# GothiProCoder/OCR-System

Hardware: AMD Instinct MI355X
Metric: pages/sec end-to-end det+rec, A4@200DPI (higher is better)
Workload: dtype bf16; 1 GPU; end-to-end det+rec, batch=64 A4@200DPI pages per GPU (BASELINE configs[3]); pages_per_gpu=64, global_batch=64, lines_last_step=3279, pages_gathered_last_step=64, parallelism=pages sharded dp1, 1 all-gather/step, ranks=1, input=pages pre-decoded (uint8 RGB) and resident in HBM when the timed region starts, det_sub_batch=64

## Files before the change

### ocr-system_amd/csrc/capi.hip

```cpp
#include <cstdlib>
#include <cstring>
#include <new>

#include "../../include/lumina_ocr.h"
#include "dbpost.h"
#include "deskew.h"
#include "engine.h"
#include "marks.h"
#include "barcodes.h"
#include "qrcodes.h"
#include "datamatrix.h"
#include "aztec.h"
#include "ops.h"
#include "orient.h"
#include "compose.h"
#include "resize.h"
#include "runs.h"
#include "jpeg.h"
#include "jpegdec.h"
#include "lzw.h"
#include "jp2dec.h"
#include "pngdec.h"
#include "vp8dec.h"
#include "webpdec.h"
// ... 94 lines not shown
    if (!eng) return 1;
    eng->device = device;
    int ndev = 0;
    if (hipGetDeviceCount(&ndev) != hipSuccess || device < 0 || device >= ndev) {
        eng->err = "no HIP device " + std::to_string(device) + " (device count " + std::to_string(ndev) + ")";
        *out = eng;
        return 2;
    }
    if (hipSetDevice(device) != hipSuccess) { eng->err = "hipSetDevice failed"; *out = eng; return 2; }
    if (const char* e = getenv("LUMINA_RING_ORIENT")) eng->ring_orient = atoi(e) < 0 ? -1 : (atoi(e) != 0);
    if (getenv("LUMINA_CONV_NO_RING")) eng->conv_ring = false;
    if (getenv("LUMINA_BLOCKED")) eng->blocked_layout = atoi(getenv("LUMINA_BLOCKED")) != 0;
    *out = eng;
    return 0;
}

void lumina_ocr_destroy(lumina_ocr_t* h) {
    if (!h) return;
    (void)hipSetDevice(h->device);
    delete h;
}

const char* lumina_ocr_last_error(const lumina_ocr_t* h) { return h ? h->err.c_str() : "null handle"; }

int lumina_ocr_set_option(lumina_ocr_t* h, const char* key, int value) {
    if (!h || !key) return 1;
    if (!strcmp(key, "det_sub_batch")) h->det_sub_batch = value > 0 ? value : 1;
    else if (!strcmp(key, "rec_sub_batch")) h->rec_sub_batch = value > 0 ? value : 1;
    else if (!strcmp(key, "cls_sub_batch")) h->cls_sub_batch = value > 0 ? value : 1;
    else if (!strcmp(key, "keep_taps")) h->keep_taps = value < 0 || value > 2 ? 0 : value;
    else if (!strcmp(key, "time_convs")) h->time_convs = value != 0;
    else if (!strcmp(key, "fuse_head")) h->fuse_head = value != 0;
    else if (!strcmp(key, "fuse_mb")) h->fuse_mb = value != 0;
    else if (!strcmp(key, "fuse_pool")) h->fuse_pool = value != 0;
    else if (!strcmp(key, "fuse_stem")) h->fuse_stem = value != 0;
    else if (!strcmp(key, "fpn_multi")) h->fpn_multi = value != 0;
    else if (!strcmp(key, "fpn_compose")) h->fpn_compose = value != 0;
    else if (!strcmp(key, "fuse_short")) h->fuse_short = value != 0;
    else if (!strcmp(key, "conv_ring")) h->conv_ring = value != 0;
    else if (!strcmp(key, "blocked_layout")) h->blocked_layout = value != 0;
    else if (!strcmp(key, "conv_big_min")) h->conv_big_min = value >= 0 ? value : 1024;
    else if (!strcmp(key, "ring_orient")) h->ring_orient = value < 0 ? -1 : (value != 0);
    else if (!strcmp(key, "post_group")) h->post_group = value > 0 ? value : 1;
    else if (!strcmp(key, "tail_group")) h->tail_group = value > 0 ? value : 0;
    else if (!strcmp(key, "svtr_f16")) h->svtr_f16 = value < 0 ? -1 : (value != 0);
    else if (!strcmp(key, "png_sub_batch_mb")) h->pd_sub_batch_mb = value > 0 ? value : 1;
    else if (!strcmp(key, "webp_sub_batch_mb")) h->wp_sub_batch_mb = value > 0 ? value : 1;
    else if (!strcmp(key, "jp2_sub_batch_mb")) h->jp_sub_batch_mb = value > 0 ? value : 1;
    else if (!strcmp(key, "conv2d_variant")) h->conv2d_variant = value < 0 || value > 2 ? 0 : value;
    else return locr_fail(h, "set_option: unknown key", key);
    return 0;
}

int lumina_ocr_load_det_weights(lumina_ocr_t* h, const void* blob, size_t nbytes) {
    if (!h || !blob) return 1;
    BIND(h);
    API_TRY return eng_load_det(h, blob, nbytes); API_CATCH(h)
}
int lumina_ocr_load_rec_weights(lumina_ocr_t* h, const void* blob, size_t nbytes) {
    if (!h || !blob) return 1;
    BIND(h);
    API_TRY return eng_load_rec(h, blob, nbytes); API_CATCH(h)
}
int lumina_ocr_num_classes(const lumina_ocr_t* h) { return h ? h->num_classes : 0; }

int lumina_ocr_normalize(lumina_ocr_t* h, const uint8_t* img_dev, int n, int height, int width, int hp, int wp, const float scale[3],
// ... 967 lines not shown
```

### ocr-system_amd/csrc/engine.h

```cpp
#pragma once
#include <map>
#include <memory>
#include <string>
#include <type_traits>
#include <vector>

#include "common.h"
#include "conv_mfma.h"
#include "mbconv.h"
#include "svtr.h"

struct Tensor4 {
    bf16_t* p = nullptr;
    int n = 0, h = 0, w = 0, c = 0;
    bool blk = false;
    int n_src = 0; const bf16_t* xs[4] = {nullptr, nullptr, nullptr, nullptr}; int xs_shift[4] = {0, 0, 0, 0};
    int xs_c[4] = {0, 0, 0, 0}, xs_cs[4] = {0, 0, 0, 0};
    int src_c(int k) const { return xs_c[k] ? xs_c[k] : c / n_src; }
    int src_cs(int k) const { return xs_cs[k] ? xs_cs[k] : src_c(k); }
    size_t elems() const { return (size_t)n * h * w * c; }
};

struct ConvLayer {
    std::string name;
// ... 49 lines not shown
inline hipError_t mem_alloc(PinnedMem* m, size_t bytes) { void* p = nullptr; hipError_t e = hipHostMalloc(&p, bytes, hipHostMallocDefault); m->reset(p); return e; }

template <class Mem> struct Growable {
    Mem mem;
    size_t cap = 0;
    uint8_t* get() const { return static_cast<uint8_t*>(mem.get()); }
    hipError_t reserve(size_t bytes, hipEvent_t in_use = nullptr) {
        if (bytes <= cap) return hipSuccess;
        hipError_t e = in_use ? hipEventSynchronize(in_use) : hipDeviceSynchronize();
        if (e != hipSuccess) return e;
        mem.reset(); cap = 0;
        if ((e = mem_alloc(&mem, bytes)) != hipSuccess) return e;
        cap = bytes;
        return hipSuccess;
    }
};

struct LaunchRecord { Event e0, e1; double flop, bytes; std::string layer, kernel; };

struct HostBlobTensor { int dtype; std::vector<int> dims; const uint8_t* data; size_t nbytes; };

struct lumina_ocr {
    int device = 0;
    std::string err;
    bool det_loaded = false;
    std::map<std::string, ConvLayer> det;
    bf16_t* stem_wpk = nullptr; float* stem_bias = nullptr;
    bool rec_loaded = false;
    int num_classes = 0, ctc_ntiles = 0;
    bf16_t* rstem_wpk = nullptr; float* rstem_bias = nullptr;
    std::vector<RecBlock> rblocks;
    ConvLayer rconv2, xproj[2];
    bf16_t* whh[2] = {nullptr, nullptr};
    bf16_t* ctc_wpk = nullptr; float* ctc_bias = nullptr;
    SvtrModel svtr;
    bool cls_loaded = false;
    bf16_t* cstem_wpk = nullptr; float* cstem_bias = nullptr;
    std::vector<RecBlock> cblocks;
    ConvLayer cconv2;
    float *cls_fc_w = nullptr, *cls_fc_b = nullptr;
    Growable<DeviceMem> ws;
    Arena arena;
    std::vector<DeviceMem> owned;
    bf16_t* zeros = nullptr;
    int det_sub_batch = 16, rec_sub_batch = 4096, cls_sub_batch = 4096, post_group = 64;
    int tail_group = 16;
    std::map<std::string, Tensor4> taps;
    int keep_taps = 0;
    bool fuse_head = true;
    bool fuse_pool = true;
    int conv_big_min = 1024;
    bool blocked_layout = true;
    bool conv_ring = true;
    int svtr_f16 = -1;
    int conv2d_variant = 0;
    int ring_orient = -1;
    bool fuse_short = true;
    bool fpn_compose = true;
    bool fpn_multi = true;
    bool fuse_stem = true;
    bool fuse_mb = true;
    bool time_convs = false;
    std::vector<LaunchRecord> launches;
    struct Coeffs { int ksize = 0; int* bounds = nullptr; int* kk = nullptr; std::shared_ptr<std::vector<int>> bounds_host; };
    std::map<std::pair<int, int>, Coeffs> coeff_cache;
    Growable<DeviceMem> aux;
    Growable<DeviceMem> sums;
    int jd_last_passes = 0;
    struct Staging { Growable<PinnedMem> buf; Event uploaded; };
    Staging jd_stage[2];
    int jd_stage_next = 0;
    Staging pd_stage;
    int pd_sub_batch_mb = 768;
    Staging jp_stage;
    Staging wp_stage;
    int wp_sub_batch_mb = 2048;
    int jp_sub_batch_mb = 4096;
    float* dk_trig = nullptr; short* dk_wtab = nullptr;
    Staging pc_stage;
    Growable<DeviceMem> pc_table;
};

int locr_fail(lumina_ocr* eng, const char* what, const char* detail);
bool parse_blob(lumina_ocr* eng, const void* blob, size_t n, std::map<std::string, HostBlobTensor>* out);

int eng_load_det(lumina_ocr* eng, const void* blob, size_t n);
int eng_load_rec(lumina_ocr* eng, const void* blob, size_t n);
int eng_det_forward(lumina_ocr* eng, const uint8_t* pages, int B, int H, int W, int Hp, int Wp, bf16_t* prob, hipStream_t st);
int eng_rec_forward(lumina_ocr* eng, const uint8_t* crops, const int* widths, int N, int* idx, float* prob, hipStream_t st);
int eng_load_svtr(lumina_ocr* eng, const void* blob, size_t n);
int eng_load_cls(lumina_ocr* eng, const void* blob, size_t n);
int eng_cls_forward(lumina_ocr* eng, const uint8_t* crops, const int* widths, int N, float thresh, int* label, float* score, int* flip, hipStream_t st);
int eng_svtr_forward(lumina_ocr* eng, const uint8_t* crops, const int* widths, int N, int* idx, float* prob, hipStream_t st);
int eng_ws_reserve(lumina_ocr* eng, size_t bytes);
// ... 19 lines not shown
```

### ocr-system_amd/csrc/engine.hip

```cpp
#include "engine.h"

#include <cstdlib>
#include <cstring>

#include "ops.h"
#include "stem_conv.h"

int locr_fail(lumina_ocr* eng, const char* what, const char* detail) {
    if (eng) eng->err = std::string(what) + ": " + (detail ? detail : "");
    return 1;
}

#define RUN(expr) do { if ((expr) != 0) return 1; } while (0)

#include <mutex>
#include <set>
hipError_t locr_dyn_lds(const void* kernel, int bytes) {
    static std::mutex mu;
    static std::set<std::pair<int, const void*>> done;
    int dev = 0;
    hipError_t e = hipGetDevice(&dev);
    if (e != hipSuccess) return e;
    std::lock_guard<std::mutex> lk(mu);
    if (done.count({dev, kernel})) return hipSuccess;
    e = hipFuncSetAttribute(kernel, hipFuncAttributeMaxDynamicSharedMemorySize, bytes);
    if (e == hipSuccess) done.insert({dev, kernel});
    return e;
}

bool parse_blob(lumina_ocr* eng, const void* blob, size_t n, std::map<std::string, HostBlobTensor>* out) {
    const uint8_t* b = static_cast<const uint8_t*>(blob);
    if (n < 12 || memcmp(b, "LOCW", 4) != 0) { locr_fail(eng, "parse_blob", "bad magic"); return false; }
    uint32_t ver, cnt;
    memcpy(&ver, b + 4, 4); memcpy(&cnt, b + 8, 4);
    if (ver != 1) { locr_fail(eng, "parse_blob", "unsupported version"); return false; }
    size_t off = 12;
    for (uint32_t i = 0; i < cnt; ++i) {
        if (off + 2 > n) { locr_fail(eng, "parse_blob", "truncated"); return false; }
// ... 591 lines not shown
        if (!make_dw(eng, m, p + ".dw", B.k, B.exp, cp16(B.exp), &B.dw)) return locr_fail(eng, "dw", p.c_str());
        {
            const HostBlobTensor *w, *b;
            if (!get_wb(eng, m, p + ".expand", &w, &b)) return 1;
            const int ec = cp16(B.exp), cc = cp16(B.cin);
            std::vector<bf16_t> padded((size_t)ec * cc, 0), packed(mbconv_expand_packed_elems(ec, cc));
            const bf16_t* src = reinterpret_cast<const bf16_t*>(w->data);
            for (int r = 0; r < B.exp; ++r) memcpy(&padded[(size_t)r * cc], &src[(size_t)r * B.cin], sizeof(bf16_t) * B.cin);
            mbconv_pack_expand(padded.data(), ec, cc, packed.data());
            std::vector<float> bias((size_t)((ec + 31) / 32) * 32, 0.f);
            memcpy(bias.data(), b->data, sizeof(float) * B.exp);
            B.we_pk = static_cast<bf16_t*>(eng_upload(eng, packed.data(), packed.size() * sizeof(bf16_t)));
            B.be_pk = static_cast<float*>(eng_upload(eng, bias.data(), bias.size() * sizeof(float)));
            if (!B.we_pk || !B.be_pk) return locr_fail(eng, "upload", (p + ".expand (fused)").c_str());
        }
        if (B.se && !make_se(eng, m, p, B.exp, cp16(B.exp), B.se_mid, &B.sel)) return 1;
        if (!make_conv(eng, m, p + ".project", 1, 1, B.exp, B.cout, cp16(B.exp), cp16(B.cout), ACT_NONE, &B.project)) return 1;
        cin = B.cout;
    }
    return 0;
}

int eng_load_rec(lumina_ocr* eng, const void* blob, size_t n) {
    std::map<std::string, HostBlobTensor> m;
    if (!parse_blob(eng, blob, n, &m)) return 1;
    LOCR_CHECK(hipSetDevice(eng->device));
    const double scale = 0.5;
    const int c0 = make_div(16 * scale);
    RUN(load_stem(eng, m, "rec.conv1", c0, &eng->rstem_wpk, &eng->rstem_bias));
    static const int sh[11] = {1, 2, 1, 2, 1, 1, 1, 1, 2, 1, 1};
    if (load_mv3_blocks(eng, m, "rec", scale, sh, c0, &eng->rblocks)) return 1;
    const int cin = eng->rblocks.back().cout;
    if (!make_conv(eng, m, "rec.conv2", 1, 1, cin, 288, cp16(cin), 288, ACT_HSWISH, &eng->rconv2)) return 1;
    const int Hh = 96;
    for (int l = 0; l < 2; ++l) {
        const int din = l == 0 ? 288 : 2 * Hh;
        const std::string pf = "lstm.l" + std::to_string(l) + ".fw", pb = "lstm.l" + std::to_string(l) + ".bw";
        auto wf = m.find(pf + ".w_ih"), wb = m.find(pb + ".w_ih"), bf = m.find(pf + ".b"), bb = m.find(pb + ".b");
        auto hf = m.find(pf + ".w_hh"), hb = m.find(pb + ".w_hh");
        if (wf == m.end() || wb == m.end() || bf == m.end() || bb == m.end() || hf == m.end() || hb == m.end())
            return locr_fail(eng, "lstm tensors missing", pf.c_str());
        if (wf->second.dims[0] != 4 * Hh || wf->second.dims[1] != din || hf->second.dims[1] != Hh) return locr_fail(eng, "lstm shape", pf.c_str());
        std::vector<uint8_t> wcat(wf->second.nbytes + wb->second.nbytes), bcat(bf->second.nbytes + bb->second.nbytes);
        memcpy(wcat.data(), wf->second.data, wf->second.nbytes); memcpy(wcat.data() + wf->second.nbytes, wb->second.data, wb->second.nbytes);
        memcpy(bcat.data(), bf->second.data, bf->second.nbytes); memcpy(bcat.data() + bf->second.nbytes, bb->second.data, bb->second.nbytes);
        std::map<std::string, HostBlobTensor> mm;
        mm["x.w"] = HostBlobTensor{1, {8 * Hh, 1, 1, din}, wcat.data(), wcat.size()};
        mm["x.b"] = HostBlobTensor{0, {8 * Hh}, bcat.data(), bcat.size()};
        if (!make_conv(eng, mm, "x", 1, 1, din, 8 * Hh, din, 8 * Hh, ACT_NONE, &eng->xproj[l])) return 1;
        eng->xproj[l].name = "lstm.l" + std::to_string(l) + ".xproj";
        std::vector<uint8_t> hcat(hf->second.nbytes + hb->second.nbytes);
        memcpy(hcat.data(), hf->second.data, hf->second.nbytes); memcpy(hcat.data() + hf->second.nbytes, hb->second.data, hb->second.nbytes);
        eng->whh[l] = static_cast<bf16_t*>(eng_upload(eng, hcat.data(), hcat.size()));
        if (!eng->whh[l]) return locr_fail(eng, "upload", "whh");
    }
    RUN(load_ctc_head(eng, m, "ctc.fc", 2 * Hh, 0, &eng->num_classes, &eng->ctc_ntiles, &eng->ctc_wpk, &eng->ctc_bias));
    eng->rec_loaded = true;
    return 0;
}

#define LAUNCH(name, expr)                                                                                        \
    do {                                                                                                          \
        if (!dry) {                                                                                               \
            if (eng->arena.overflow) return ws_null(eng, name);                                                   \
            hipError_t _e = (expr); if (_e != hipSuccess) return locr_fail(eng, name, hipGetErrorString(_e));     \
        }                                                                                                         \
    } while (0)

static int run_mv3_block(lumina_ocr* eng, const RecBlock& B, const std::string& name, Tensor4* x, hipStream_t st) {
    const bool dry = eng->arena.counting();
    const int N = x->n;
    const int ho = (x->h + 2 * (B.k / 2) - B.k) / B.stride_h + 1;
    MbParams mp{};
    mp.we = B.we_pk; mp.be = B.be_pk; mp.wd = B.dw.w; mp.bd = B.dw.bias;
    mp.N = N; mp.H = x->h; mp.W = x->w; mp.cin = x->c; mp.expc = cp16(B.exp); mp.Ho = ho; mp.act = B.act;
    const bool fused_mb = eng->fuse_mb && mbconv_supported(mp, B.k, B.stride_h);
    Tensor4 e1{};
    if (!fused_mb || dry) e1 = ws_tensor(eng, N, x->h, x->w, cp16(B.exp));
    Tensor4 d = ws_tensor(eng, N, ho, x->w, cp16(B.exp));
    float* pool = B.se ? eng->arena.take<float>((size_t)N * mb_strips(x->w) * d.c) : nullptr;
    if (fused_mb) {
        mp.x = x->p; mp.d = d.p; mp.pool = pool;
        if (!dry && x->p && d.p) {
            LaunchTimer tm(eng, st);
            LAUNCH("mbconv", mbconv_launch(mp, B.k, B.stride_h, st));
            const double opx = (double)N * ho * x->w, ipx = (double)N * x->h * x->w;
            tm.done(name + ".expand+dw", "mbconv_kernel<" + std::to_string(B.k) + "," + std::to_string(B.stride_h) + "," + std::to_string(B.act) + ">",
                    2.0 * ipx * x->c * mp.expc + 2.0 * opx * B.k * B.k * mp.expc, 2.0 * (ipx * x->c + opx * mp.expc));
        }
    } else {
        RUN(eng_run_conv(eng, B.expand, *x, &e1, st, ConvCall().flat_gemm()));
        LAUNCH("dwconv", dwconv_launch(e1.p, B.dw.w, B.dw.bias, d.p, N, e1.h, e1.w, e1.c, B.k, B.stride_h, B.act, st));
        if (B.se) LAUNCH("se_pool", se_pool_launch(d.p, pool, N, d.h, d.w, d.c, st));
    }
    const bf16_t* se_gate_ptr = nullptr;
    if (B.se) {
        bf16_t* gate = eng->arena.take<bf16_t>((size_t)N * d.c);
        LAUNCH("se_fc", se_fc_launch(pool, mb_strips(d.w), B.sel.w1, B.sel.b1, B.sel.w2, B.sel.b2, gate, N, d.h * d.w, d.c, B.sel.mid, st));
        se_gate_ptr = gate;
    }
    Tensor4 o = ws_tensor(eng, N, d.h, d.w, cp16(B.cout));
    RUN(eng_run_conv(eng, B.project, d, &o, st, ConvCall().flat_gemm().residual(B.res ? x : nullptr).gated(se_gate_ptr)));
    tap(eng, name.c_str(), o);
    *x = o;
    return 0;
}

static int rec_forward_sub(lumina_ocr* eng, const uint8_t* crops, const int* widths, int N, int* idx, float* prob, hipStream_t st) {
    const bool dry = eng->arena.counting();
    const int T = 80;
    Tensor4 x = ws_tensor(eng, N, 16, 160, 16);
    RUN(run_stem(eng, "rec.conv1", crops, widths, N, 32, 320, eng->rstem_wpk, eng->rstem_bias, ACT_HSWISH, STEM_SCALE_PM1, STEM_SHIFT_PM1, x, st));
    tap(eng, "rec.conv1", x);
    for (size_t bi = 0; bi < eng->rblocks.size(); ++bi) RUN(run_mv3_block(eng, eng->rblocks[bi], "rec.b" + std::to_string(bi), &x, st));
    Tensor4 f = ws_tensor(eng, N, x.h, x.w, 288);
    RUN(eng_run_conv(eng, eng->rconv2, x, &f, st, ConvCall().flat_gemm())); tap(eng, "rec.conv2", f);
    Tensor4 seq = ws_tensor(eng, N, 1, T, 288);
    LAUNCH("rec.pool", maxpool_launch(f.p, seq.p, N, f.h, f.w, 288, 2, 2, 0, 1, T, st));
    tap(eng, "rec.feat", seq);
    for (int l = 0; l < 2; ++l) {
        Tensor4 xp = ws_tensor(eng, N, 1, T, 8 * 96);
        RUN(eng_run_conv(eng, eng->xproj[l], seq, &xp, st, ConvCall().flat_gemm()));
        Tensor4 hs = ws_tensor(eng, N, 1, T, 2 * 96);
        {
            LaunchTimer tm(eng, st, !dry);
            LAUNCH("lstm", lstm_recurrent_launch(xp.p, eng->whh[l], hs.p, N, T, st));
            tm.done("lstm.l" + std::to_string(l), "lstm_kernel", 2.0 * N * T * 2 * 96 * 384, 2.0 * N * T * (768 + 192));
        }
        tap(eng, l == 0 ? "lstm.l0" : "lstm.l1", hs);
        seq = hs;
    }
    if (!dry) {
        CtcFcParams cp{};
        cp.seq = seq.p; cp.wpk = eng->ctc_wpk; cp.bias = eng->ctc_bias; cp.out_idx = idx; cp.out_prob = prob;
        cp.M = N * T; cp.K = 192; cp.C = eng->num_classes; cp.ntiles = eng->ctc_ntiles;
        LaunchTimer tm(eng, st);
        LAUNCH("ctc_fc_argmax", ctc_fc_argmax_launch(cp, st));
        tm.done("ctc.fc+argmax", "ctc_fc_argmax_kernel<0>", 2.0 * cp.M * cp.K * cp.C, 2.0 * cp.M * cp.K + 8.0 * cp.M + 2.0 * cp.K * cp.C);
    }
    return 0;
}

int eng_rec_forward(lumina_ocr* eng, const uint8_t* crops, const int* widths, int N, int* idx, float* prob, hipStream_t st) {
    if (!eng->rec_loaded) return locr_fail(eng, "rec_forward", "rec weights not loaded");
    if (N <= 0) return 0;
    LOCR_CHECK(hipSetDevice(eng->device));
    return forward_sub_batched(eng, N, eng->rec_sub_batch < N ? eng->rec_sub_batch : N, [&](int b0, int nb) {
        return rec_forward_sub(eng, crops + (size_t)b0 * 32 * 320 * 3, widths ? widths + b0 : nullptr, nb, idx + (size_t)b0 * 80, prob + (size_t)b0 * 80, st);
    });
}

int eng_load_cls(lumina_ocr* eng, const void* blob, size_t n) {
    std::map<std::string, HostBlobTensor> m;
    if (!parse_blob(eng, blob, n, &m)) return 1;
    LOCR_CHECK(hipSetDevice(eng->device));
    eng->cls_loaded = false;
    const double scale = 0.35;
    const int c0 = make_div(16 * scale);
    RUN(load_stem(eng, m, "cls.conv1", c0, &eng->cstem_wpk, &eng->cstem_bias));
    static const int sh[11] = {2, 2, 1, 2, 1, 1, 1, 1, 2, 1, 1};
// ... 238 lines not shown
```

### ocr-system_amd/csrc/ops.h

```cpp
#pragma once
#include "common.h"

hipError_t maxpool_launch(const bf16_t* x, bf16_t* y, int N, int H, int W, int C, int k, int s, int pad, int Ho, int Wo, hipStream_t st);

hipError_t dwconv_launch(const bf16_t* x, const bf16_t* w, const float* bias, bf16_t* y, int N, int H, int W, int C, int k,
                         int sh, int act, hipStream_t st);

hipError_t se_fc_launch(const float* pool, int strips, const bf16_t* w1, const float* b1, const bf16_t* w2, const float* b2, bf16_t* gate,
                        int N, int HW, int C, int mid, hipStream_t st);
hipError_t se_scale_launch(const bf16_t* x, const bf16_t* gate, bf16_t* y, int N, int HW, int C, hipStream_t st);

hipError_t lstm_recurrent_launch(const bf16_t* xproj, const bf16_t* whh, bf16_t* out, int N, int T, hipStream_t st);

struct CtcFcParams {
    const bf16_t* seq;
    const bf16_t* wpk;
    const float* bias;
    float* part_max; int* part_idx; float* part_sum;
    int* out_idx; float* out_prob;
    int M, K, C, ntiles;
    int f16;
};
size_t ctc_packed_weight_elems(int C, int K);
void pack_ctc_weights(const bf16_t* w , int C, int K, bf16_t* out);
hipError_t ctc_fc_argmax_launch(const CtcFcParams& p, hipStream_t st);

hipError_t cls_head_launch(const bf16_t* feat, const float* w, const float* b, int N, int P, int C, int Cs, float thresh, int* label, float* score,
                           int* flip, bf16_t* logits_bf16, hipStream_t st);

hipError_t ctc_collapse_launch(const int* idx, const float* prob, int* text, int* len, float* score, int N, int T, hipStream_t st);
hipError_t ctc_words_launch(const int* idx, const float* prob, const int* quads, const int* widths, const int* flip, int space_id, int* text,
                            int* len, float* score, int* word_quads, int* word_span, float* word_score, int* word_count, int N, int T,
                            hipStream_t st);
```

### ocr-system_amd/csrc/ops.hip

```cpp
#include "ops.h"
#include "../../include/lumina_ocr.h"

#include <type_traits>

#include <cstdlib>

namespace {

__device__ __forceinline__ void unpack8(const uint4 v, float* f) {
    f[0] = __uint_as_float(v.x << 16); f[1] = __uint_as_float(v.x & 0xFFFF0000u);
    f[2] = __uint_as_float(v.y << 16); f[3] = __uint_as_float(v.y & 0xFFFF0000u);
    f[4] = __uint_as_float(v.z << 16); f[5] = __uint_as_float(v.z & 0xFFFF0000u);
    f[6] = __uint_as_float(v.w << 16); f[7] = __uint_as_float(v.w & 0xFFFF0000u);
}
__device__ __forceinline__ uint4 pack8(const float* f) {
    uint4 v;
    v.x = pack_bf16x2(f[0], f[1]); v.y = pack_bf16x2(f[2], f[3]);
    v.z = pack_bf16x2(f[4], f[5]); v.w = pack_bf16x2(f[6], f[7]);
    return v;
}

__global__ void maxpool_kernel(const bf16_t* x, bf16_t* y, int N, int H, int W, int C, int k, int s, int pad, int Ho, int Wo) {
    const int cg = C >> 3;
    const size_t total = (size_t)N * Ho * Wo * cg;
// ... 102 lines not shown
    for (int m = tid; m < mid; m += 256) {
        float s = 0.f;
        for (int c = 0; c < C; ++c) s = s + bf16_to_f32(w1[(size_t)m * C + c]) * mean[c];
        hid[m] = bf16_to_f32(f32_to_bf16(fmaxf(s + b1[m], 0.f)));
    }
    __syncthreads();
    for (int c = tid; c < C; c += 256) {
        float s = 0.f;
        for (int m = 0; m < mid; ++m) s = s + bf16_to_f32(w2[(size_t)c * mid + m]) * hid[m];
        gate[(size_t)n * C + c] = f32_to_bf16(apply_act(s + b2[c], ACT_HSIGMOID));
    }
}

__global__ void se_scale_kernel(const bf16_t* x, const bf16_t* gate, bf16_t* y, int N, int HW, int C) {
    const int cg = C >> 3;
    const size_t total = (size_t)N * HW * cg;
    for (size_t i = (size_t)blockIdx.x * blockDim.x + threadIdx.x; i < total; i += (size_t)gridDim.x * blockDim.x) {
        const int c8 = (int)(i % cg);
        const int n = (int)(i / ((size_t)HW * cg));
        float f[8], g[8];
        unpack8(*reinterpret_cast<const uint4*>(x + i * 8), f);
        unpack8(*reinterpret_cast<const uint4*>(gate + (size_t)n * C + c8 * 8), g);
#pragma unroll
        for (int j = 0; j < 8; ++j) f[j] = f[j] * g[j];
        *reinterpret_cast<uint4*>(y + i * 8) = pack8(f);
    }
}

constexpr int LH = 96, LSEQ = 32, LPITCH = 208;

__device__ __forceinline__ float fast_sigmoid(float x) { return __builtin_amdgcn_rcpf(1.f + __builtin_amdgcn_exp2f(-1.4426950408889634f * x)); }
__device__ __forceinline__ float fast_tanh(float x) { return 2.f * fast_sigmoid(2.f * x) - 1.f; }

__global__ __launch_bounds__(192) void lstm_kernel(const bf16_t* xproj, const bf16_t* whh, bf16_t* out, int N, int T) {
    __shared__ __attribute__((aligned(16))) unsigned char hbuf[2][LSEQ * LPITCH];
    const int tid = threadIdx.x, lane = tid & 63, u = tid >> 6, r = lane & 31, h = lane >> 5;
    const int dir = blockIdx.x & 1, n0 = (blockIdx.x >> 1) * LSEQ;
    const int seq = n0 + r;
    const bool valid = seq < N;
    const int sq = valid ? seq : N - 1;
    bf16x8_t afr[4][6];
#pragma unroll
    for (int g = 0; g < 4; ++g)
#pragma unroll
        for (int ks = 0; ks < 6; ++ks)
            afr[g][ks] = *reinterpret_cast<const bf16x8_t*>(whh + ((size_t)dir * 4 * LH + g * LH + 32 * u + r) * LH + ks * 16 + h * 8);
    for (int i = tid; i < 2 * LSEQ * LPITCH / 16; i += 192) reinterpret_cast<uint4*>(&hbuf[0][0])[i] = make_uint4(0, 0, 0, 0);
    float c[16];
#pragma unroll
    for (int j = 0; j < 16; ++j) c[j] = 0.f;
    const size_t xrow = (size_t)sq * T;
    const int xcol = dir * 4 * LH + 32 * u + 4 * h;
    uint2 xq[4][4];
    {
        const int t = dir ? T - 1 : 0;
#pragma unroll
        for (int g = 0; g < 4; ++g)
#pragma unroll
            for (int q = 0; q < 4; ++q) xq[g][q] = *reinterpret_cast<const uint2*>(xproj + (xrow + t) * (8 * LH) + xcol + g * LH + 8 * q);
    }
    __syncthreads();
    int cur = 0;
    for (int step = 0; step < T; ++step) {
        const int t = dir ? (T - 1 - step) : step;
        f32x16_t acc[4];
#pragma unroll
        for (int g = 0; g < 4; ++g)
// ... 2 lines not shown
                acc[g][4 * q + 0] = __uint_as_float(xq[g][q].x << 16); acc[g][4 * q + 1] = __uint_as_float(xq[g][q].x & 0xFFFF0000u);
                acc[g][4 * q + 2] = __uint_as_float(xq[g][q].y << 16); acc[g][4 * q + 3] = __uint_as_float(xq[g][q].y & 0xFFFF0000u);
            }
        if (step + 1 < T) {
            const int tn = dir ? (t - 1) : (t + 1);
#pragma unroll
            for (int g = 0; g < 4; ++g)
#pragma unroll
                for (int q = 0; q < 4; ++q) xq[g][q] = *reinterpret_cast<const uint2*>(xproj + (xrow + tn) * (8 * LH) + xcol + g * LH + 8 * q);
        }
#pragma unroll
        for (int ks = 0; ks < 6; ++ks) {
            const bf16x8_t bfr = *reinterpret_cast<const bf16x8_t*>(&hbuf[cur][r * LPITCH + (ks * 16 + h * 8) * 2]);
#pragma unroll
            for (int g = 0; g < 4; ++g) acc[g] = __builtin_amdgcn_mfma_f32_32x32x16_bf16(afr[g][ks], bfr, acc[g], 0, 0, 0);
        }
        bf16_t* orow = out + ((size_t)sq * T + t) * (2 * LH) + dir * LH + 32 * u + 4 * h;
#pragma unroll
        for (int q = 0; q < 4; ++q) {
            float hn[4];
#pragma unroll
            for (int e = 0; e < 4; ++e) {
                const int j = 4 * q + e;
                const float ig = fast_sigmoid(acc[0][j]), fg = fast_sigmoid(acc[1][j]), gg = fast_tanh(acc[2][j]), og = fast_sigmoid(acc[3][j]);
                c[j] = fg * c[j] + ig * gg;
                hn[e] = og * fast_tanh(c[j]);
            }
            uint2 o;
            o.x = pack_bf16x2(hn[0], hn[1]);
            o.y = pack_bf16x2(hn[2], hn[3]);
            *reinterpret_cast<uint2*>(&hbuf[cur ^ 1][r * LPITCH + (32 * u + 8 * q + 4 * h) * 2]) = o;
            if (valid) *reinterpret_cast<uint2*>(orow + 8 * q) = o;
        }
        __syncthreads();
        cur ^= 1;
    }
}

constexpr int CT_NT = 2;
constexpr int CT_ROWS = 4 * 32, CT_BN = 32 * CT_NT, CT_K = 192, CT_KSTEPS = CT_K / 16;
constexpr int CT_W_ITEMS = CT_BN * (CT_K / 8);
constexpr int CT_WIT = CT_W_ITEMS / 256, CT_WBYTES = CT_W_ITEMS * 16;
constexpr int CT_BIAS_SLOTS = 4;
constexpr size_t CT_LDS = 2 * (size_t)CT_WBYTES;
static_assert(CT_W_ITEMS % 256 == 0 && CT_BN * sizeof(float) / 16 <= 64, "the staging below has no remainder loop");

typedef _Float16 ctc_f16x8_t __attribute__((ext_vector_type(8)));
template <int DT>
__global__ __launch_bounds__(256, 2) void ctc_fc_argmax_kernel(const CtcFcParams p) {
    typedef typename std::conditional<DT == 1, ctc_f16x8_t, bf16x8_t>::type frag_t;
    extern __shared__ __attribute__((aligned(16))) unsigned char smem[];
    __shared__ __attribute__((aligned(16))) float sB[CT_BIAS_SLOTS * CT_BN];
    unsigned char* sW = smem;
    const int tid = threadIdx.x, lane = tid & 63, wave = tid >> 6, r = lane & 31, h = lane >> 5;
    const int row0 = blockIdx.x * CT_ROWS;
    const int last = p.ntiles - 1;
    constexpr float LOG2E = 1.4426950408889634f;

    frag_t arow[CT_KSTEPS];
    {
        const int row = row0 + wave * 32 + r;
        const frag_t* src = reinterpret_cast<const frag_t*>(p.seq + (size_t)row * CT_K) + h;
#pragma unroll
        for (int kc = 0; kc < CT_KSTEPS; ++kc) {
            frag_t v = {};
            if (row < p.M) v = src[2 * kc];
// ... 254 lines not shown
hipError_t dwconv_launch(const bf16_t* x, const bf16_t* w, const float* bias, bf16_t* y, int N, int H, int W, int C, int k,
                         int sh, int act, hipStream_t st) {
    const int Ho = (H + 2 * (k / 2) - k) / sh + 1;
    const size_t total = (size_t)N * Ho * ((W + 3) / 4) * (C / 8);
    if (total > 0x7fffffffull || (k != 3 && k != 5)) return hipErrorInvalidValue;
    const size_t lds = ((size_t)k * k * C + C) * sizeof(float);
    if (lds > 60 * 1024) return hipErrorInvalidValue;
    const dim3 g(grid_for(total));
#define DW(K_, A_) hipLaunchKernelGGL((dwconv_kernel<K_, A_>), g, dim3(256), lds, st, x, w, bias, y, N, H, W, C, sh, Ho)
#define DW_ACT(K_)                                                     \
    switch (act) {                                                     \
        case ACT_NONE: DW(K_, ACT_NONE); break;                        \
        case ACT_RELU: DW(K_, ACT_RELU); break;                        \
        case ACT_HSWISH: DW(K_, ACT_HSWISH); break;                    \
        default: return hipErrorInvalidValue;                          \
    }
    if (k == 3) { DW_ACT(3) } else { DW_ACT(5) }
#undef DW_ACT
#undef DW
    return hipGetLastError();
}

hipError_t se_fc_launch(const float* pool, int strips, const bf16_t* w1, const float* b1, const bf16_t* w2, const float* b2, bf16_t* gate,
                        int N, int HW, int C, int mid, hipStream_t st) {
    hipLaunchKernelGGL(se_fc_kernel, dim3(N), dim3(256), ((size_t)C + mid) * sizeof(float), st, pool, strips, w1, b1, w2, b2, gate, HW, C, mid);
    return hipGetLastError();
}

hipError_t se_scale_launch(const bf16_t* x, const bf16_t* gate, bf16_t* y, int N, int HW, int C, hipStream_t st) {
    hipLaunchKernelGGL(se_scale_kernel, dim3(grid_for((size_t)N * HW * (C / 8))), dim3(256), 0, st, x, gate, y, N, HW, C);
    return hipGetLastError();
}

hipError_t lstm_recurrent_launch(const bf16_t* xproj, const bf16_t* whh, bf16_t* out, int N, int T, hipStream_t st) {
    hipLaunchKernelGGL(lstm_kernel, dim3(((N + LSEQ - 1) / LSEQ) * 2), dim3(192), 0, st, xproj, whh, out, N, T);
    return hipGetLastError();
}

size_t ctc_packed_weight_elems(int C, int K) { return (size_t)((C + CT_BN - 1) / CT_BN) * CT_BN * K; }

void pack_ctc_weights(const bf16_t* w, int C, int K, bf16_t* out) {
    const int ntiles = (C + CT_BN - 1) / CT_BN, npl = K / 8;
    for (int t = 0; t < ntiles; ++t)
        for (int c = 0; c < npl; ++c)
            for (int n = 0; n < CT_BN; ++n)
                for (int j = 0; j < 8; ++j) {
                    const int cls = t * CT_BN + n;
                    out[(((size_t)t * npl + c) * CT_BN + n) * 8 + j] = cls < C ? w[(size_t)cls * K + c * 8 + j] : (bf16_t)0;
                }
}

hipError_t ctc_fc_argmax_launch(const CtcFcParams& p, hipStream_t st) {
    if (p.K != CT_K || p.ntiles < 1 || p.M < 1) return hipErrorInvalidValue;
    const size_t lds = CT_LDS;
    if (p.f16) {
        { hipError_t e = locr_dyn_lds(reinterpret_cast<const void*>(ctc_fc_argmax_kernel<1>), (int)CT_LDS); if (e != hipSuccess) return e; }
        hipLaunchKernelGGL(ctc_fc_argmax_kernel<1>, dim3((p.M + CT_ROWS - 1) / CT_ROWS), dim3(256), lds, st, p);
    } else {
        { hipError_t e = locr_dyn_lds(reinterpret_cast<const void*>(ctc_fc_argmax_kernel<0>), (int)CT_LDS); if (e != hipSuccess) return e; }
        hipLaunchKernelGGL(ctc_fc_argmax_kernel<0>, dim3((p.M + CT_ROWS - 1) / CT_ROWS), dim3(256), lds, st, p);
    }
    return hipGetLastError();
}

hipError_t ctc_collapse_launch(const int* idx, const float* prob, int* text, int* len, float* score, int N, int T, hipStream_t st) {
    if (T > 128) return hipErrorInvalidValue;
    hipLaunchKernelGGL(ctc_collapse_kernel, dim3(N), dim3(64), 0, st, idx, prob, text, len, score, T);
    return hipGetLastError();
// ... 19 lines not shown
```

Before: 1690 pages/sec.

## Add sequence GEMM for rec conv2+pool and LSTM input projection; widen LSTM to 12 waves

Adds a dedicated MFMA sequence GEMM kernel. It fuses the recognizer's 1x1 conv2 (hswish) with the following 2x2 max-pool, so the full-resolution feature map is never written. The same kernel replaces the generic conv path for the LSTM input projections. The LSTM recurrent kernel is reworked to use 12 waves per block instead of 3, so each wave handles one 8-unit slice per step, cutting the serial per-step work and raising parallelism. The cost is more block-level synchronisation per step and extra weight copies in a new packed layout.

```diff
diff --git a/ocr-system_amd/csrc/capi.hip b/ocr-system_amd/csrc/capi.hip
--- a/ocr-system_amd/csrc/capi.hip
+++ b/ocr-system_amd/csrc/capi.hip
@@ -150,6 +150,10 @@
     else if (!strcmp(key, "time_convs")) h->time_convs = value != 0;
     else if (!strcmp(key, "fuse_head")) h->fuse_head = value != 0;
     else if (!strcmp(key, "fuse_mb")) h->fuse_mb = value != 0;
+    else if (!strcmp(key, "fuse_xproj")) h->fuse_xproj = value != 0;
+    else if (!strcmp(key, "fuse_conv2_pool")) h->fuse_conv2_pool = value != 0;
+    else if (!strcmp(key, "lstm_waves")) h->lstm_waves = value == 3 ? 3 : 12;
+    else if (!strcmp(key, "seq_gemm_min")) h->seq_gemm_min = value >= 0 ? value : 128;
     else if (!strcmp(key, "fuse_pool")) h->fuse_pool = value != 0;
     else if (!strcmp(key, "fuse_stem")) h->fuse_stem = value != 0;
     else if (!strcmp(key, "fpn_multi")) h->fpn_multi = value != 0;
diff --git a/ocr-system_amd/csrc/engine.h b/ocr-system_amd/csrc/engine.h
--- a/ocr-system_amd/csrc/engine.h
+++ b/ocr-system_amd/csrc/engine.h
@@ -105,6 +105,7 @@
     std::vector<RecBlock> rblocks;
     ConvLayer rconv2, xproj[2];
     bf16_t* whh[2] = {nullptr, nullptr};
+    bf16_t *xproj_spk[2] = {nullptr, nullptr}, *rconv2_spk = nullptr;
     bf16_t* ctc_wpk = nullptr; float* ctc_bias = nullptr;
     SvtrModel svtr;
     bool cls_loaded = false;
@@ -133,6 +134,10 @@
     bool fpn_multi = true;
     bool fuse_stem = true;
     bool fuse_mb = true;
+    bool fuse_xproj = true;
+    bool fuse_conv2_pool = true;
+    int lstm_waves = 12;
+    int seq_gemm_min = 128;
     bool time_convs = false;
     std::vector<LaunchRecord> launches;
     struct Coeffs { int ksize = 0; int* bounds = nullptr; int* kk = nullptr; std::shared_ptr<std::vector<int>> bounds_host; };
diff --git a/ocr-system_amd/csrc/engine.hip b/ocr-system_amd/csrc/engine.hip
--- a/ocr-system_amd/csrc/engine.hip
+++ b/ocr-system_amd/csrc/engine.hip
@@ -4,6 +4,7 @@
 #include <cstring>
 
 #include "ops.h"
+#include "seq_gemm.h"
 #include "stem_conv.h"
 
 int locr_fail(lumina_ocr* eng, const char* what, const char* detail) {
@@ -661,6 +662,13 @@
     if (load_mv3_blocks(eng, m, "rec", scale, sh, c0, &eng->rblocks)) return 1;
     const int cin = eng->rblocks.back().cout;
     if (!make_conv(eng, m, "rec.conv2", 1, 1, cin, 288, cp16(cin), 288, ACT_HSWISH, &eng->rconv2)) return 1;
+    eng->rconv2_spk = nullptr;
+    if (cin == 48) {
+        std::vector<bf16_t> spk(seq_gemm_packed_elems(288, cin));
+        seq_gemm_pack_weights(reinterpret_cast<const bf16_t*>(m.find("rec.conv2.w")->second.data), 288, cin, spk.data());
+        eng->rconv2_spk = static_cast<bf16_t*>(eng_upload(eng, spk.data(), spk.size() * sizeof(bf16_t)));
+        if (!eng->rconv2_spk) return locr_fail(eng, "upload", "rec.conv2 (seq_gemm)");
+    }
     const int Hh = 96;
     for (int l = 0; l < 2; ++l) {
         const int din = l == 0 ? 288 : 2 * Hh;
@@ -678,6 +686,12 @@
         mm["x.b"] = HostBlobTensor{0, {8 * Hh}, bcat.data(), bcat.size()};
         if (!make_conv(eng, mm, "x", 1, 1, din, 8 * Hh, din, 8 * Hh, ACT_NONE, &eng->xproj[l])) return 1;
         eng->xproj[l].name = "lstm.l" + std::to_string(l) + ".xproj";
+        {
+            std::vector<bf16_t> spk(seq_gemm_packed_elems(8 * Hh, din));
+            seq_gemm_pack_weights(reinterpret_cast<const bf16_t*>(wcat.data()), 8 * Hh, din, spk.data());
+            eng->xproj_spk[l] = static_cast<bf16_t*>(eng_upload(eng, spk.data(), spk.size() * sizeof(bf16_t)));
+            if (!eng->xproj_spk[l]) return locr_fail(eng, "upload", "xproj (seq_gemm)");
+        }
         std::vector<uint8_t> hcat(hf->second.nbytes + hb->second.nbytes);
         memcpy(hcat.data(), hf->second.data, hf->second.nbytes); memcpy(hcat.data() + hf->second.nbytes, hb->second.data, hb->second.nbytes);
         eng->whh[l] = static_cast<bf16_t*>(eng_upload(eng, hcat.data(), hcat.size()));
@@ -742,19 +756,41 @@
     RUN(run_stem(eng, "rec.conv1", crops, widths, N, 32, 320, eng->rstem_wpk, eng->rstem_bias, ACT_HSWISH, STEM_SCALE_PM1, STEM_SHIFT_PM1, x, st));
     tap(eng, "rec.conv1", x);
     for (size_t bi = 0; bi < eng->rblocks.size(); ++bi) RUN(run_mv3_block(eng, eng->rblocks[bi], "rec.b" + std::to_string(bi), &x, st));
-    Tensor4 f = ws_tensor(eng, N, x.h, x.w, 288);
-    RUN(eng_run_conv(eng, eng->rconv2, x, &f, st, ConvCall().flat_gemm())); tap(eng, "rec.conv2", f);
+    auto seq_gemm = [&](const char* layer, const ConvLayer& L, const bf16_t* spk, const Tensor4& in, Tensor4& out, int epi) -> int {
+        SeqGemmParams sp{};
+        sp.x = in.p; sp.wpk = spk; sp.bias = L.bias; sp.y = out.p;
+        sp.M = N * T; sp.K = in.c; sp.Cout = out.c; sp.T = T; sp.epi = epi;
+        if (dry) return 0;
+        LaunchTimer tm(eng, st);
+        LAUNCH(layer, seq_gemm_launch(sp, st));
+        const double px = (double)N * in.h * in.w;
+        tm.done(layer, seq_gemm_kernel_name(sp), 2.0 * px * in.c * out.c, 2.0 * (px * in.c + (double)sp.M * out.c + (double)in.c * out.c));
+        return 0;
+    };
+    const bool seq_fills = (N * T + 127) / 128 >= eng->seq_gemm_min;
+    const bool pool_fused = seq_fills && eng->fuse_conv2_pool && eng->keep_taps != 1 && eng->rconv2_spk != nullptr && eng->rconv2.cfg.bn == 64 &&
+                            x.h == 2 && x.w == 2 * T && x.c == 48;
+    Tensor4 f{};
+    if (!pool_fused || dry) f = ws_tensor(eng, N, x.h, x.w, 288);
     Tensor4 seq = ws_tensor(eng, N, 1, T, 288);
-    LAUNCH("rec.pool", maxpool_launch(f.p, seq.p, N, f.h, f.w, 288, 2, 2, 0, 1, T, st));
+    if (pool_fused) {
+        RUN(seq_gemm("rec.conv2+pool", eng->rconv2, eng->rconv2_spk, x, seq, SEQ_POOL4));
+    } else {
+        RUN(eng_run_conv(eng, eng->rconv2, x, &f, st, ConvCall().flat_gemm())); tap(eng, "rec.conv2", f);
+        LAUNCH("rec.pool", maxpool_launch(f.p, seq.p, N, f.h, f.w, 288, 2, 2, 0, 1, T, st));
+    }
     tap(eng, "rec.feat", seq);
     for (int l = 0; l < 2; ++l) {
         Tensor4 xp = ws_tensor(eng, N, 1, T, 8 * 96);
-        RUN(eng_run_conv(eng, eng->xproj[l], seq, &xp, st, ConvCall().flat_gemm()));
+        if (seq_fills && eng->fuse_xproj && eng->xproj_spk[l] != nullptr && eng->xproj[l].cfg.bn == 64 && (seq.c == 288 || seq.c == 192))
+            RUN(seq_gemm(eng->xproj[l].name.c_str(), eng->xproj[l], eng->xproj_spk[l], seq, xp, SEQ_STORE));
+        else
+            RUN(eng_run_conv(eng, eng->xproj[l], seq, &xp, st, ConvCall().flat_gemm()));
         Tensor4 hs = ws_tensor(eng, N, 1, T, 2 * 96);
         {
             LaunchTimer tm(eng, st, !dry);
-            LAUNCH("lstm", lstm_recurrent_launch(xp.p, eng->whh[l], hs.p, N, T, st));
-            tm.done("lstm.l" + std::to_string(l), "lstm_kernel", 2.0 * N * T * 2 * 96 * 384, 2.0 * N * T * (768 + 192));
+            LAUNCH("lstm", lstm_recurrent_launch(xp.p, eng->whh[l], hs.p, N, T, st, eng->lstm_waves));
+            tm.done("lstm.l" + std::to_string(l), eng->lstm_waves == 3 ? "lstm3_kernel" : "lstm_kernel", 2.0 * N * T * 2 * 96 * 384, 2.0 * N * T * (768 + 192));
         }
         tap(eng, l == 0 ? "lstm.l0" : "lstm.l1", hs);
         seq = hs;
diff --git a/ocr-system_amd/csrc/ops.h b/ocr-system_amd/csrc/ops.h
--- a/ocr-system_amd/csrc/ops.h
+++ b/ocr-system_amd/csrc/ops.h
@@ -10,7 +10,7 @@
                         int N, int HW, int C, int mid, hipStream_t st);
 hipError_t se_scale_launch(const bf16_t* x, const bf16_t* gate, bf16_t* y, int N, int HW, int C, hipStream_t st);
 
-hipError_t lstm_recurrent_launch(const bf16_t* xproj, const bf16_t* whh, bf16_t* out, int N, int T, hipStream_t st);
+hipError_t lstm_recurrent_launch(const bf16_t* xproj, const bf16_t* whh, bf16_t* out, int N, int T, hipStream_t st, int waves = 12);
 
 struct CtcFcParams {
     const bf16_t* seq;
diff --git a/ocr-system_amd/csrc/ops.hip b/ocr-system_amd/csrc/ops.hip
--- a/ocr-system_amd/csrc/ops.hip
+++ b/ocr-system_amd/csrc/ops.hip
@@ -158,7 +158,7 @@
 __device__ __forceinline__ float fast_sigmoid(float x) { return __builtin_amdgcn_rcpf(1.f + __builtin_amdgcn_exp2f(-1.4426950408889634f * x)); }
 __device__ __forceinline__ float fast_tanh(float x) { return 2.f * fast_sigmoid(2.f * x) - 1.f; }
 
-__global__ __launch_bounds__(192) void lstm_kernel(const bf16_t* xproj, const bf16_t* whh, bf16_t* out, int N, int T) {
+__global__ __launch_bounds__(192) void lstm3_kernel(const bf16_t* xproj, const bf16_t* whh, bf16_t* out, int N, int T) {
     __shared__ __attribute__((aligned(16))) unsigned char hbuf[2][LSEQ * LPITCH];
     const int tid = threadIdx.x, lane = tid & 63, u = tid >> 6, r = lane & 31, h = lane >> 5;
     const int dir = blockIdx.x & 1, n0 = (blockIdx.x >> 1) * LSEQ;
@@ -227,6 +227,64 @@
             *reinterpret_cast<uint2*>(&hbuf[cur ^ 1][r * LPITCH + (32 * u + 8 * q + 4 * h) * 2]) = o;
             if (valid) *reinterpret_cast<uint2*>(orow + 8 * q) = o;
         }
+        __syncthreads();
+        cur ^= 1;
+    }
+}
+
+__global__ __launch_bounds__(768) void lstm_kernel(const bf16_t* xproj, const bf16_t* whh, bf16_t* out, int N, int T) {
+    __shared__ __attribute__((aligned(16))) unsigned char hbuf[2][LSEQ * LPITCH];
+    const int tid = threadIdx.x, lane = tid & 63, w = tid >> 6, r = lane & 31, h = lane >> 5;
+    const int dir = blockIdx.x & 1, n0 = (blockIdx.x >> 1) * LSEQ;
+    const int seq = n0 + r;
+    const bool valid = seq < N;
+    const int sq = valid ? seq : N - 1;
+    bf16x8_t afr[6];
+#pragma unroll
+    for (int ks = 0; ks < 6; ++ks)
+        afr[ks] = *reinterpret_cast<const bf16x8_t*>(whh + ((size_t)dir * 4 * LH + (r >> 3) * LH + 8 * w + (r & 7)) * LH + ks * 16 + h * 8);
+    for (int i = tid; i < 2 * LSEQ * LPITCH / 16; i += 768) reinterpret_cast<uint4*>(&hbuf[0][0])[i] = make_uint4(0, 0, 0, 0);
+    float c[4] = {0.f, 0.f, 0.f, 0.f};
+    const size_t xrow = (size_t)sq * T;
+    const int xcol = dir * 4 * LH + 8 * w + 4 * h;
+    uint2 xq[4];
+    {
+        const int t = dir ? T - 1 : 0;
+#pragma unroll
+        for (int q = 0; q < 4; ++q) xq[q] = *reinterpret_cast<const uint2*>(xproj + (xrow + t) * (8 * LH) + xcol + q * LH);
+    }
+    __syncthreads();
+    int cur = 0;
+    for (int step = 0; step < T; ++step) {
+        const int t = dir ? (T - 1 - step) : step;
+        f32x16_t acc;
+#pragma unroll
+        for (int q = 0; q < 4; ++q) {
+            acc[4 * q + 0] = __uint_as_float(xq[q].x << 16); acc[4 * q + 1] = __uint_as_float(xq[q].x & 0xFFFF0000u);
+            acc[4 * q + 2] = __uint_as_float(xq[q].y << 16); acc[4 * q + 3] = __uint_as_float(xq[q].y & 0xFFFF0000u);
+        }
+        if (step + 1 < T) {
+            const int tn = dir ? (t - 1) : (t + 1);
+#pragma unroll
+            for (int q = 0; q < 4; ++q) xq[q] = *reinterpret_cast<const uint2*>(xproj + (xrow + tn) * (8 * LH) + xcol + q * LH);
+        }
+#pragma unroll
+        for (int ks = 0; ks < 6; ++ks) {
+            const bf16x8_t bfr = *reinterpret_cast<const bf16x8_t*>(&hbuf[cur][r * LPITCH + (ks * 16 + h * 8) * 2]);
+            acc = __builtin_amdgcn_mfma_f32_32x32x16_bf16(afr[ks], bfr, acc, 0, 0, 0);
+        }
+        float hn[4];
+#pragma unroll
+        for (int e = 0; e < 4; ++e) {
+            const float ig = fast_sigmoid(acc[e]), fg = fast_sigmoid(acc[4 + e]), gg = fast_tanh(acc[8 + e]), og = fast_sigmoid(acc[12 + e]);
+            c[e] = fg * c[e] + ig * gg;
+            hn[e] = og * fast_tanh(c[e]);
+        }
+        uint2 o;
+        o.x = pack_bf16x2(hn[0], hn[1]);
+        o.y = pack_bf16x2(hn[2], hn[3]);
+        *reinterpret_cast<uint2*>(&hbuf[cur ^ 1][r * LPITCH + (8 * w + 4 * h) * 2]) = o;
+        if (valid) *reinterpret_cast<uint2*>(out + ((size_t)sq * T + t) * (2 * LH) + dir * LH + 8 * w + 4 * h) = o;
         __syncthreads();
         cur ^= 1;
     }
@@ -547,8 +605,11 @@
     return hipGetLastError();
 }
 
-hipError_t lstm_recurrent_launch(const bf16_t* xproj, const bf16_t* whh, bf16_t* out, int N, int T, hipStream_t st) {
-    hipLaunchKernelGGL(lstm_kernel, dim3(((N + LSEQ - 1) / LSEQ) * 2), dim3(192), 0, st, xproj, whh, out, N, T);
+hipError_t lstm_recurrent_launch(const bf16_t* xproj, const bf16_t* whh, bf16_t* out, int N, int T, hipStream_t st, int waves) {
+    if (N < 1 || T < 1 || (waves != 3 && waves != 12)) return hipErrorInvalidValue;
+    const dim3 grid(((N + LSEQ - 1) / LSEQ) * 2);
+    if (waves == 3) hipLaunchKernelGGL(lstm3_kernel, grid, dim3(192), 0, st, xproj, whh, out, N, T);
+    else hipLaunchKernelGGL(lstm_kernel, grid, dim3(768), 0, st, xproj, whh, out, N, T);
     return hipGetLastError();
 }
 
diff --git a/ocr-system_amd/csrc/seq_gemm.h b/ocr-system_amd/csrc/seq_gemm.h
--- /dev/null
+++ b/ocr-system_amd/csrc/seq_gemm.h
@@ -0,0 +1,23 @@
+#pragma once
+#include "common.h"
+
+enum SeqGemmEpi : int {
+    SEQ_STORE = 0,
+    SEQ_POOL4 = 1,
+};
+
+struct SeqGemmParams {
+    const bf16_t* x;
+    const bf16_t* wpk;
+    const float* bias;
+    bf16_t* y;
+    int M, K, Cout;
+    int T;
+    int epi;
+};
+
+size_t seq_gemm_packed_elems(int cout, int K);
+void seq_gemm_pack_weights(const bf16_t* w , int cout, int K, bf16_t* out);
+bool seq_gemm_supported(const SeqGemmParams& p);
+hipError_t seq_gemm_launch(const SeqGemmParams& p, hipStream_t st);
+const char* seq_gemm_kernel_name(const SeqGemmParams& p);
diff --git a/ocr-system_amd/csrc/seq_gemm.hip b/ocr-system_amd/csrc/seq_gemm.hip
--- /dev/null
+++ b/ocr-system_amd/csrc/seq_gemm.hip
@@ -0,0 +1,184 @@
+#include "seq_gemm.h"
+
+namespace {
+
+constexpr int SG_ROWS = 4 * 32, SG_BN = 64, SG_NT = 2, SG_BIAS_SLOTS = 4;
+
+template <int K, int EPI>
+__global__ __launch_bounds__(256, 2) void seq_gemm_kernel(const SeqGemmParams p) {
+    constexpr int KSTEPS = K / 16, NM = EPI == SEQ_POOL4 ? 4 : 1;
+    constexpr int W_ITEMS = SG_BN * (K / 8), WIT = (W_ITEMS + 255) / 256, WBYTES = W_ITEMS * 16;
+    static_assert(K % 16 == 0 && W_ITEMS % 64 == 0, "whole k steps; the ragged last staging pass ends on a wave boundary");
+    extern __shared__ __attribute__((aligned(16))) unsigned char smem[];
+    __shared__ __attribute__((aligned(16))) float sB[SG_BIAS_SLOTS * SG_BN];
+    unsigned char* sW = smem;
+    const int tid = threadIdx.x, lane = tid & 63, wave = tid >> 6, r = lane & 31, h = lane >> 5;
+    const int ntiles = (p.Cout + SG_BN - 1) / SG_BN, last = ntiles - 1;
+    const int row = blockIdx.x * SG_ROWS + wave * 32 + r;
+    const bool valid = row < p.M;
+
+    bf16x8_t arow[NM][KSTEPS];
+#pragma unroll
+    for (int m = 0; m < NM; ++m) {
+        size_t pix = (size_t)row;
+        if constexpr (EPI == SEQ_POOL4) {
+            const int n = row / p.T, t = row - n * p.T;
+            pix = ((size_t)(n * 2 + (m >> 1))) * (2 * p.T) + 2 * t + (m & 1);
+        }
+        const bf16x8_t* src = reinterpret_cast<const bf16x8_t*>(p.x + pix * K) + h;
+#pragma unroll
+        for (int kc = 0; kc < KSTEPS; ++kc) {
+            bf16x8_t v = {};
+            if (valid) v = src[2 * kc];
+            arow[m][kc] = v;
+        }
+    }
+
+    uint4 breg = make_uint4(0, 0, 0, 0);
+    auto stage = [&](int tile, int slot) {
+        const uint4* src = reinterpret_cast<const uint4*>(p.wpk) + (size_t)tile * W_ITEMS + tid;
+        unsigned char* dst = sW + (slot & 1) * WBYTES + (tid - lane) * 16;
+#pragma unroll
+        for (int it = 0; it < WIT; ++it)
+            if (W_ITEMS % 256 == 0 || tid - lane + 256 * it < W_ITEMS)
+                __builtin_amdgcn_global_load_lds((const __attribute__((address_space(1))) void*)(src + 256 * it),
+                                                 (__attribute__((address_space(3))) void*)(dst + 256 * it * 16), 16, 0, 0);
+        if (tid < SG_BN / 4) breg = reinterpret_cast<const uint4*>(p.bias + (size_t)tile * SG_BN)[tid];
+    };
+    auto landed = [&](int slot) {
+        asm volatile("s_waitcnt vmcnt(0)" ::: "memory");
+        if (tid < SG_BN / 4) reinterpret_cast<uint4*>(sB + (slot & (SG_BIAS_SLOTS - 1)) * SG_BN)[tid] = breg;
+        __syncthreads();
+    };
+
+    auto mma = [&](f32x16_t (&acc)[NM][SG_NT], int t) {
+        const unsigned char* w = sW + (t & 1) * WBYTES + (h * SG_BN + r) * 16;
+        bf16x8_t wf[2][SG_NT];
+#pragma unroll
+        for (int nt = 0; nt < SG_NT; ++nt) wf[0][nt] = *reinterpret_cast<const bf16x8_t*>(w + nt * 32 * 16);
+#pragma unroll
+        for (int kc = 0; kc < KSTEPS; ++kc) {
+            if (kc + 1 < KSTEPS) {
+#pragma unroll
+                for (int nt = 0; nt < SG_NT; ++nt)
+                    wf[(kc + 1) & 1][nt] = *reinterpret_cast<const bf16x8_t*>(w + (2 * (kc + 1) * SG_BN + nt * 32) * 16);
+            }
+#pragma unroll
+            for (int m = 0; m < NM; ++m)
+#pragma unroll
+                for (int nt = 0; nt < SG_NT; ++nt) {
+                    const f32x16_t c = kc == 0 ? f32x16_t{} : acc[m][nt];
+                    acc[m][nt] = __builtin_amdgcn_mfma_f32_32x32x16_bf16(wf[kc & 1][nt], arow[m][kc], c, 0, 0, 0);
+                }
+        }
+    };
+    auto store = [&](const f32x16_t (&acc)[NM][SG_NT], int t) {
+        const float* bt = sB + (t & (SG_BIAS_SLOTS - 1)) * SG_BN + 4 * h;
+        bf16_t* yrow = p.y + (size_t)row * p.Cout + t * SG_BN + 8 * h;
+#pragma unroll
+        for (int nt = 0; nt < SG_NT; ++nt)
+#pragma unroll
+            for (int gp = 0; gp < 2; ++gp) {
+                float o[8];
+#pragma unroll
+                for (int g = 0; g < 2; ++g) {
+                    const int q = 2 * gp + g;
+                    const f32x4_t b = __builtin_bit_cast(f32x4_t, *reinterpret_cast<const bf16x8_t*>(bt + nt * 32 + 8 * q));
+#pragma unroll
+                    for (int e = 0; e < 4; ++e) {
+                        if constexpr (EPI == SEQ_POOL4) {
+                            float mx = -3.0e38f;
+#pragma unroll
+                            for (int m = 0; m < NM; ++m)
+                                mx = fmaxf(mx, bf16_to_f32(f32_to_bf16(apply_act(acc[m][nt][4 * q + e] + b[e], ACT_HSWISH))));
+                            o[4 * g + e] = mx;
+                        } else {
+                            o[4 * g + e] = acc[0][nt][4 * q + e] + b[e];
+                        }
+                    }
+                }
+                const uint32_t q0x = pack_bf16x2(o[0], o[1]), q0y = pack_bf16x2(o[2], o[3]);
+                const uint32_t q1x = pack_bf16x2(o[4], o[5]), q1y = pack_bf16x2(o[6], o[7]);
+                const auto sx = __builtin_amdgcn_permlane32_swap(q0x, q1x, false, false);
+                const auto sy = __builtin_amdgcn_permlane32_swap(q0y, q1y, false, false);
+                const int co = nt * 32 + 16 * gp;
+                if (valid && t * SG_BN + co + 8 * h < p.Cout) *reinterpret_cast<uint4*>(yrow + co) = make_uint4(sx[0], sy[0], sx[1], sy[1]);
+            }
+    };
+
+    stage(0, 0);
+    landed(0);
+    if constexpr (EPI == SEQ_POOL4) {
+        f32x16_t acc[NM][SG_NT];
+        for (int t = 0; t < ntiles; ++t) {
+            stage(min(t + 1, last), t + 1);
+            mma(acc, t);
+            store(acc, t);
+            landed(t + 1);
+        }
+    } else {
+        auto step = [&](f32x16_t (&accc)[NM][SG_NT], const f32x16_t (&acce)[NM][SG_NT], int t) {
+            stage(min(t + 1, last), t + 1);
+            store(acce, t - 1);
+            mma(accc, t);
+            landed(t + 1);
+        };
+        f32x16_t acc0[NM][SG_NT], acc1[NM][SG_NT];
+        stage(min(1, last), 1);
+        mma(acc0, 0);
+        landed(1);
+        int t = 1;
+        for (; t + 1 < ntiles; t += 2) {
+            step(acc1, acc0, t);
+            step(acc0, acc1, t + 1);
+        }
+        if (t < ntiles) {
+            step(acc1, acc0, t);
+            store(acc1, t);
+        } else {
+            store(acc0, last);
+        }
+    }
+}
+
+template <int K, int EPI>
+hipError_t launch(const SeqGemmParams& p, hipStream_t st) {
+    const int lds = 2 * SG_BN * (K / 8) * 16;
+    const void* fn = reinterpret_cast<const void*>(seq_gemm_kernel<K, EPI>);
+    { hipError_t e = locr_dyn_lds(fn, lds); if (e != hipSuccess) return e; }
+    hipLaunchKernelGGL((seq_gemm_kernel<K, EPI>), dim3((p.M + SG_ROWS - 1) / SG_ROWS), dim3(256), lds, st, p);
+    return hipGetLastError();
+}
+
+}
+
+size_t seq_gemm_packed_elems(int cout, int K) { return (size_t)((cout + SG_BN - 1) / SG_BN) * SG_BN * K; }
+
+void seq_gemm_pack_weights(const bf16_t* w, int cout, int K, bf16_t* out) {
+    const int ntiles = (cout + SG_BN - 1) / SG_BN, npl = K / 8;
+    for (int t = 0; t < ntiles; ++t)
+        for (int c = 0; c < npl; ++c)
+            for (int n = 0; n < SG_BN; ++n)
+                for (int j = 0; j < 8; ++j) {
+                    const int co = t * SG_BN + n;
+                    out[(((size_t)t * npl + c) * SG_BN + n) * 8 + j] = co < cout ? w[(size_t)co * K + c * 8 + j] : (bf16_t)0;
+                }
+}
+
+bool seq_gemm_supported(const SeqGemmParams& p) {
+    if (p.M < 1 || p.Cout < 8 || p.Cout % 8 != 0 || (size_t)p.M * 4 > 0x7fffffffull) return false;
+    if (p.epi == SEQ_STORE) return p.K == 288 || p.K == 192;
+    if (p.epi == SEQ_POOL4) return p.K == 48 && p.T >= 1 && p.M % p.T == 0;
+    return false;
+}
+
+hipError_t seq_gemm_launch(const SeqGemmParams& p, hipStream_t st) {
+    if (!seq_gemm_supported(p)) return hipErrorInvalidValue;
+    if (p.epi == SEQ_POOL4) return launch<48, SEQ_POOL4>(p, st);
+    return p.K == 288 ? launch<288, SEQ_STORE>(p, st) : launch<192, SEQ_STORE>(p, st);
+}
+
+const char* seq_gemm_kernel_name(const SeqGemmParams& p) {
+    if (p.epi == SEQ_POOL4) return "seq_gemm_kernel<48,1>";
+    return p.K == 288 ? "seq_gemm_kernel<288,0>" : "seq_gemm_kernel<192,0>";
+}
```

After: 1720 pages/sec, median of 6. 1.8% higher.
